# Ai00-X/ai00_server

Hardware: NVIDIA H100
Metric: decode tokens/s RWKV-6-World-7B fp16 batch=16 (higher is better)
Workload: dtype f16

## Files before the change

ai00_server_b200/csrc/wkv.cuh:

```cuda
#pragma once
#include "common.cuh"

namespace b200 {

constexpr int WKV_N = 64;
constexpr float GN_EPS = 64e-5f;

struct WkvParams {
    int version;
    int ld;
    MetaView meta;
    float* state;
    int H;
    const float* r;
    const float* k;
    const float* v;
    const float* g;
    const float* w;
    const float* w_static;
    const float* u;
    const float* lnx_w;
    const float* lnx_b;
    const float* a;
    const float* nu;
    float* v_first;
    int layer0;
    const float* k_k;
    const float* k_a;
    const float* r_k;
    __half* out;
    int kq_tile;
    const __half* wd2t;
    const float* decay_bias;
    const __half* d1;
    int d1_kq;
    int Dd;
    unsigned long long* trace;
};

struct WkvShared {
    float r[WKV_N], k[WKV_N], v[WKV_N], w[WKV_N], b[WKV_N], o[WKV_N];
    float red[4];
};

template <int VER, int KC = 8, bool SPLIT = false>
__device__ __forceinline__ void wkv_slot(const WkvParams& p, const int h, const int t0, const int nt, float (&m)[4][KC],
                                         WkvShared& sm, const float* w_local, const int lt0, const float* pre = nullptr,
                                         const int pre_stride = 0, const float* statics = nullptr) {
    const int tid = (int)threadIdx.x;
    constexpr int LANES = WKV_N / KC;
    const int ig = tid / LANES;
    const int j4 = tid % LANES;
    const int ch = h * WKV_N;
    float u4[KC];
#pragma unroll
    for (int f = 0; f < KC; ++f) u4[f] = 0.f;
    if (VER != 7) {
#pragma unroll
        for (int f = 0; f < KC; ++f) u4[f] = statics ? statics[2 * WKV_N + j4 * KC + f] : p.u[ch + j4 * KC + f];
    }
    for (int tt = 0; tt < nt; ++tt) {
        const int t = t0 + tt;
        const size_t row = (size_t)t * p.ld + ch;
        if (tid < WKV_N) {
            const int c = tid;
            const int pi = (lt0 + tt) * WKV_N + c;
            float r = pre ? pre[pi] : p.r[row + c];
            float k = pre ? pre[pre_stride + pi] : p.k[row + c];
            float v = pre ? pre[2 * pre_stride + pi] : p.v[row + c];
            float w;
            if (VER == 5) w = p.w_static[ch + c];
            else if (w_local) w = w_local[pi];
            else w = pre ? pre[4 * pre_stride + pi] : p.w[row + c];
            if (VER == 7) {
                const float a = pre ? pre[5 * pre_stride + pi] : p.a[row + c];
                float kk = k * p.k_k[ch + c];
                float ss = warp_sum(kk * kk);
                if ((tid & 31) == 0) sm.red[tid >> 5] = ss;
                asm volatile("bar.sync 2, 64;" ::: "memory");
                ss = sm.red[0] + sm.red[1];
                kk = kk / fmaxf(sqrtf(ss), 1e-12f);
                k = k * (1.f + (a - 1.f) * p.k_a[ch + c]);
                if (p.layer0) p.v_first[row + c] = v;
                else v = v + (p.v_first[row + c] - v) * (pre ? pre[6 * pre_stride + pi] : p.nu[row + c]);
                float bonus = warp_sum(r * k * p.r_k[ch + c]);
                if ((tid & 31) == 0) sm.red[2 + (tid >> 5)] = bonus;
                sm.b[c] = kk * a;
                sm.o[c] = -kk;
            }
            sm.r[c] = r; sm.k[c] = k; sm.v[c] = v; sm.w[c] = w;
        }
        __syncthreads();

        float rr[KC], kk_[KC], ww[KC];
#pragma unroll
        for (int f = 0; f < KC; ++f) { rr[f] = sm.r[j4 * KC + f]; kk_[f] = sm.k[j4 * KC + f]; ww[f] = sm.w[j4 * KC + f]; }
        float o[4];
        if (VER != 7) {
#pragma unroll
            for (int e = 0; e < 4; ++e) {
                const float vv = sm.v[ig * 4 + e];
                float* me = m[e];
                float acc = 0.f;
#pragma unroll
                for (int f = 0; f < KC; ++f) {
                    const float kv = kk_[f] * vv;
                    acc += rr[f] * (u4[f] * kv + me[f]);
                    me[f] = kv + ww[f] * me[f];
                }
                o[e] = acc;
            }
        } else {
            float nk[KC], ka[KC];
#pragma unroll
            for (int f = 0; f < KC; ++f) { nk[f] = sm.o[j4 * KC + f]; ka[f] = sm.b[j4 * KC + f]; }
            float sa[4];
#pragma unroll
            for (int e = 0; e < 4; ++e) {
                const float* me = m[e];
                float s_ = 0.f;
#pragma unroll
                for (int f = 0; f < KC; f += 4) s_ += (me[f] * nk[f] + me[f + 1] * nk[f + 1]) + (me[f + 2] * nk[f + 2] + me[f + 3] * nk[f + 3]);
                sa[e] = s_;
            }
#pragma unroll
            for (int off = LANES / 2; off > 0; off >>= 1)
#pragma unroll
                for (int e = 0; e < 4; ++e) sa[e] += __shfl_xor_sync(0xffffffffu, sa[e], off);
#pragma unroll
            for (int e = 0; e < 4; ++e) {
                const float vv = sm.v[ig * 4 + e];
                float* me = m[e];
                float acc = 0.f;
#pragma unroll
                for (int f = 0; f < KC; ++f) {
                    me[f] = me[f] * ww[f] + sa[e] * ka[f] + vv * kk_[f];
                    acc += me[f] * rr[f];
                }
                o[e] = acc;
            }
        }
#pragma unroll
        for (int off = LANES / 2; off > 0; off >>= 1)
#pragma unroll
            for (int e = 0; e < 4; ++e) o[e] += __shfl_xor_sync(0xffffffffu, o[e], off);
        __syncthreads();
        if (j4 == 0) {
#pragma unroll
            for (int e = 0; e < 4; ++e) sm.o[ig * 4 + e] = o[e];
        }
        __syncthreads();

        if (tid < 32) {
            const float x0 = sm.o[tid], x1 = sm.o[tid + 32];
            const float mean = warp_sum(x0 + x1) * (1.f / WKV_N);
            const float d0 = x0 - mean, d1 = x1 - mean;
            const float var = warp_sum(d0 * d0 + d1 * d1) * (1.f / WKV_N);
            const float rstd = 1.0f / sqrtf(var + GN_EPS);
            const float lw0 = statics ? statics[tid] : p.lnx_w[ch + tid], lw1 = statics ? statics[tid + 32] : p.lnx_w[ch + tid + 32];
            const float lb0 = statics ? statics[WKV_N + tid] : p.lnx_b[ch + tid];
            const float lb1 = statics ? statics[WKV_N + tid + 32] : p.lnx_b[ch + tid + 32];
            float y0 = d0 * rstd * lw0 + lb0;
            float y1 = d1 * rstd * lw1 + lb1;
            if (VER == 7) {
                const float bonus = sm.red[2] + sm.red[3];
                y0 += bonus * sm.v[tid];
                y1 += bonus * sm.v[tid + 32];
            }
            const int gi = (lt0 + tt) * WKV_N + tid;
            y0 *= pre ? pre[3 * pre_stride + gi] : p.g[row + tid];
            y1 *= pre ? pre[3 * pre_stride + gi + 32] : p.g[row + tid + 32];
            if (SPLIT) {
                __half h0, l0, h1, l1;
                split_h(y0, h0, l0);
                split_h(y1, h1, l1);
                p.out[a16_index(t, ch + tid, p.kq_tile)] = h0;
                p.out[a16_index(t, ch + tid + 32, p.kq_tile)] = h1;
                p.out[a16_index(t + 16, ch + tid, p.kq_tile)] = l0;
                p.out[a16_index(t + 16, ch + tid + 32, p.kq_tile)] = l1;
            } else {
                p.out[a16_index(t, ch + tid, p.kq_tile)] = f2h_sat(y0);
                p.out[a16_index(t, ch + tid + 32, p.kq_tile)] = f2h_sat(y1);
            }
        }
        __syncthreads();
    }
}

constexpr int WKV_SA_THREADS = 128;
constexpr int WKV_SA_KC = 8;
constexpr int WKV_STAGE_TOK = 4;
constexpr int WKV_STAGE_ARRAYS = 7;

__host__ __device__ inline int wkv_stage_arrays(int ver, bool fold) { return ver == 7 ? 7 : ((ver == 6 && !fold) ? 5 : 4); }

__host__ __device__ inline size_t wkv_smem_bytes(int ver, bool fold, int Dd, int max_tokens, bool split = false) {
    size_t b = 0;
    (void)max_tokens;
    if (fold) b += (size_t)WKV_N * Dd * 2 + (size_t)WKV_STAGE_TOK * WKV_N * 4 + ((((size_t)WKV_STAGE_TOK * Dd * 2 * (split ? 2 : 1)) + 15) & ~(size_t)15) + 2 * WKV_N * 4;
    b += (size_t)wkv_stage_arrays(ver, fold) * WKV_STAGE_TOK * WKV_N * 4 + 3 * WKV_N * 4 + 64;
    return b;
}

template <int VER, bool SPLIT = false>
__global__ void __launch_bounds__(WKV_SA_THREADS, 7) wkv_kernel(const __grid_constant__ WkvParams p, const int max_tokens) {
    constexpr int KC = WKV_SA_KC, LANES = WKV_N / KC, NT = WKV_SA_THREADS;
    __shared__ WkvShared sm;
    extern __shared__ __align__(16) uint8_t wkv_dyn[];
    trace_stamp(p.trace, 0);
    pdl_launch_dependents();
    const int si = blockIdx.y;
    const int h = blockIdx.x;
    const int tid = threadIdx.x;
    const int ig = tid / LANES, j4 = tid % LANES;
    const int ch = h * WKV_N;
    const bool fold = (VER == 6) && p.wd2t != nullptr;
    const int Dd = fold ? p.Dd : 0;
    uint8_t* dyn = wkv_dyn;
    __half* wt = reinterpret_cast<__half*>(dyn);
    float* wl = nullptr;
    __half* ds = nullptr;
    float* part = nullptr;
    if (fold) {
        wl = reinterpret_cast<float*>(dyn + (size_t)WKV_N * Dd * 2);
        ds = reinterpret_cast<__half*>(wl + (size_t)WKV_STAGE_TOK * WKV_N);
        part = reinterpret_cast<float*>(reinterpret_cast<uint8_t*>(ds) + ((((size_t)WKV_STAGE_TOK * Dd * 2 * (SPLIT ? 2 : 1)) + 15) & ~(size_t)15));
        dyn = reinterpret_cast<uint8_t*>(part + 2 * WKV_N);
    }
    const int na = wkv_stage_arrays(VER, fold);
    float* pre_s = reinterpret_cast<float*>(dyn);
    float* statics = pre_s + na * WKV_STAGE_TOK * WKV_N;
    if (fold) {
        const uint4* src = reinterpret_cast<const uint4*>(p.wd2t + (size_t)h * WKV_N * Dd);
        uint4* dst = reinterpret_cast<uint4*>(wt);
        for (int i = tid; i < WKV_N * Dd / 8; i += NT) dst[i] = src[i];
    }
    for (int i = tid; i < 3 * WKV_N; i += NT) {
        const int a = i >> 6, c = i & (WKV_N - 1);
        float v = 0.f;
        if (a == 0) v = p.lnx_w[ch + c];
        else if (a == 1) v = p.lnx_b[ch + c];
        else if (VER != 7) v = p.u[ch + c];
        statics[i] = v;
    }
    const float bias = fold ? p.decay_bias[ch + (tid & (WKV_N - 1))] : 0.f;
    const int nslots = p.meta.nslots();
    const bool live = si < nslots;
    const int slot = live ? p.meta.slot_id()[si] : 0;
    const int t0 = live ? p.meta.slot_start()[si] : 0;
    const int nt = live ? p.meta.slot_count()[si] : 0;
    float* M = p.state + ((size_t)slot * p.H + h) * (WKV_N * WKV_N);
    float m[4][KC];
    if (live) {
#pragma unroll
        for (int e = 0; e < 4; ++e)
#pragma unroll
            for (int q = 0; q < KC / 4; ++q) {
                const float4 v4 = __ldcs(reinterpret_cast<const float4*>(M + (ig * 4 + e) * WKV_N + j4 * KC + q * 4));
                m[e][q * 4] = v4.x; m[e][q * 4 + 1] = v4.y; m[e][q * 4 + 2] = v4.z; m[e][q * 4 + 3] = v4.w;
            }
    }
    pdl_wait();
    trace_stamp(p.trace, 1);
    if (!live) return;

    const bool staged = nt <= WKV_STAGE_TOK;
    if (staged) {
        constexpr int UMAX = WKV_STAGE_ARRAYS * WKV_STAGE_TOK * WKV_N / NT;
        const int per = nt * WKV_N, total = na * per;
        const int ndd = fold ? nt * Dd : 0;
#pragma unroll
        for (int half = 0; half < 2; ++half) {
            float val[UMAX / 2];
#pragma unroll
            for (int u = 0; u < UMAX / 2; ++u) {
                const int i = tid + (half * (UMAX / 2) + u) * NT;
                val[u] = 0.f;
                if (i < total) {
                    const int a = i / per, rem = i - a * per;
                    const size_t at = (size_t)(t0 + (rem >> 6)) * p.ld + ch + (rem & (WKV_N - 1));
                    const float* src = a == 0 ? p.r : a == 1 ? p.k : a == 2 ? p.v : a == 3 ? p.g : a == 4 ? p.w : a == 5 ? p.a : p.nu;
                    if (src) val[u] = src[at];
                }
            }
#pragma unroll
            for (int u = 0; u < UMAX / 2; ++u) {
                const int i = tid + (half * (UMAX / 2) + u) * NT;
                if (i < total) {
                    const int a = i / per, rem = i - a * per;
                    pre_s[a * (WKV_STAGE_TOK * WKV_N) + rem] = val[u];
                }
            }
        }
        for (int i = tid; i < ndd; i += NT) {
            const int tt = i / Dd;
            ds[i] = p.d1[a16_index(t0 + tt, i - tt * Dd, p.d1_kq)];
        }
        if (SPLIT)
            for (int i = tid; i < ndd; i += NT) {
                const int tt = i / Dd;
                ds[WKV_STAGE_TOK * Dd + i] = p.d1[a16_index(t0 + tt + 16, i - tt * Dd, p.d1_kq)];
            }
    }

    auto fold_token = [&](const __half* dt, const int slot_tok) {
        const int c = tid & (WKV_N - 1), qk = tid >> 6;
        const int kq0 = qk * (Dd >> 1), kq1 = kq0 + (Dd >> 1);
        float acc0 = 0.f, acc1 = 0.f;
        if (SPLIT) {
            const __half* dl = dt + WKV_STAGE_TOK * Dd;
            for (int k = kq0; k < kq1; k += 2) {
                acc0 = fmaf(__half2float(wt[k * WKV_N + c]), __half2float(dt[k]) + __half2float(dl[k]), acc0);
                acc1 = fmaf(__half2float(wt[(k + 1) * WKV_N + c]), __half2float(dt[k + 1]) + __half2float(dl[k + 1]), acc1);
            }
        } else {
            for (int k = kq0; k < kq1; k += 2) {
                acc0 = fmaf(__half2float(wt[k * WKV_N + c]), __half2float(dt[k]), acc0);
                acc1 = fmaf(__half2float(wt[(k + 1) * WKV_N + c]), __half2float(dt[k + 1]), acc1);
            }
        }
        part[qk * WKV_N + c] = acc0 + acc1;
        __syncthreads();
        if (tid < WKV_N) wl[slot_tok * WKV_N + c] = expf(-expf(bias + (part[c] + part[WKV_N + c])));
    };
    if (staged || !fold) {
        if (fold)
            for (int tt = 0; tt < nt; ++tt) {
                __syncthreads();
                fold_token(ds + tt * Dd, tt);
            }
        __syncthreads();
        wkv_slot<VER, KC, SPLIT>(p, h, t0, nt, m, sm, fold ? wl : nullptr, 0, staged ? pre_s : nullptr, WKV_STAGE_TOK * WKV_N, statics);
    } else {
        for (int tt = 0; tt < nt; ++tt) {
            __syncthreads();
            for (int k = tid; k < Dd; k += NT) ds[k] = p.d1[a16_index(t0 + tt, k, p.d1_kq)];
            if (SPLIT)
                for (int k = tid; k < Dd; k += NT) ds[WKV_STAGE_TOK * Dd + k] = p.d1[a16_index(t0 + tt + 16, k, p.d1_kq)];
            __syncthreads();
            fold_token(ds, 0);
            __syncthreads();
            wkv_slot<VER, KC, SPLIT>(p, h, t0 + tt, 1, m, sm, wl, 0, nullptr, WKV_STAGE_TOK * WKV_N, statics);
        }
    }
#pragma unroll
    for (int e = 0; e < 4; ++e)
#pragma unroll
        for (int q = 0; q < KC / 4; ++q)
            __stcs(reinterpret_cast<float4*>(M + (ig * 4 + e) * WKV_N + j4 * KC + q * 4),
                   make_float4(m[e][q * 4], m[e][q * 4 + 1], m[e][q * 4 + 2], m[e][q * 4 + 3]));
    trace_stamp(p.trace, 7);
}

}
```

Baseline: 2192.

## Interleave WKV shared-memory columns and stream per-column operands to cut registers

Stores r/k/w/b and the bonus u in shared memory with a permuted column index, so each lane reads stride-LANES columns without bank conflicts. The state update now loops over columns and reads those operands from shared memory one at a time instead of holding whole per-lane arrays in registers. The staging loader becomes a rolled loop with a small buffer, and launch bounds go from 7 to 8 blocks per SM to raise occupancy. This trades more shared-memory loads inside the inner loop for lower register pressure.

```diff
diff --git a/ai00_server_b200/csrc/wkv.cuh b/ai00_server_b200/csrc/wkv.cuh
--- a/ai00_server_b200/csrc/wkv.cuh
+++ b/ai00_server_b200/csrc/wkv.cuh
@@ -5,6 +5,7 @@
 
 constexpr int WKV_N = 64;
 constexpr float GN_EPS = 64e-5f;
+constexpr int WKV_STAGE_TOK = 4;
 
 struct WkvParams {
     int version;
@@ -38,6 +39,8 @@
     unsigned long long* trace;
 };
 
+__device__ __forceinline__ int wkv_kcol(const int c) { return (c & 7) * 8 + (c >> 3); }
+
 struct WkvShared {
     float r[WKV_N], k[WKV_N], v[WKV_N], w[WKV_N], b[WKV_N], o[WKV_N];
     float red[4];
@@ -45,35 +48,30 @@
 
 template <int VER, int KC = 8, bool SPLIT = false>
 __device__ __forceinline__ void wkv_slot(const WkvParams& p, const int h, const int t0, const int nt, float (&m)[4][KC],
-                                         WkvShared& sm, const float* w_local, const int lt0, const float* pre = nullptr,
-                                         const int pre_stride = 0, const float* statics = nullptr) {
+                                         WkvShared& sm, const float* w_local, const float* pre, const bool staged,
+                                         const float* statics) {
     const int tid = (int)threadIdx.x;
     constexpr int LANES = WKV_N / KC;
     const int ig = tid / LANES;
     const int j4 = tid % LANES;
     const int ch = h * WKV_N;
-    float u4[KC];
-#pragma unroll
-    for (int f = 0; f < KC; ++f) u4[f] = 0.f;
-    if (VER != 7) {
-#pragma unroll
-        for (int f = 0; f < KC; ++f) u4[f] = statics ? statics[2 * WKV_N + j4 * KC + f] : p.u[ch + j4 * KC + f];
-    }
+    const bool fold = VER == 6 && p.wd2t != nullptr;
+    constexpr int PS = WKV_STAGE_TOK * WKV_N;
     for (int tt = 0; tt < nt; ++tt) {
         const int t = t0 + tt;
         const size_t row = (size_t)t * p.ld + ch;
         if (tid < WKV_N) {
-            const int c = tid;
-            const int pi = (lt0 + tt) * WKV_N + c;
-            float r = pre ? pre[pi] : p.r[row + c];
-            float k = pre ? pre[pre_stride + pi] : p.k[row + c];
-            float v = pre ? pre[2 * pre_stride + pi] : p.v[row + c];
+            const int c = tid, kc = wkv_kcol(c);
+            const int pi = tt * WKV_N + c;
+            float r = staged ? pre[pi] : p.r[row + c];
+            float k = staged ? pre[PS + pi] : p.k[row + c];
+            float v = staged ? pre[2 * PS + pi] : p.v[row + c];
             float w;
             if (VER == 5) w = p.w_static[ch + c];
-            else if (w_local) w = w_local[pi];
-            else w = pre ? pre[4 * pre_stride + pi] : p.w[row + c];
+            else if (fold) w = w_local[pi];
+            else w = staged ? pre[4 * PS + pi] : p.w[row + c];
             if (VER == 7) {
-                const float a = pre ? pre[5 * pre_stride + pi] : p.a[row + c];
+                const float a = staged ? pre[5 * PS + pi] : p.a[row + c];
                 float kk = k * p.k_k[ch + c];
                 float ss = warp_sum(kk * kk);
                 if ((tid & 31) == 0) sm.red[tid >> 5] = ss;
@@ -82,62 +80,55 @@
                 kk = kk / fmaxf(sqrtf(ss), 1e-12f);
                 k = k * (1.f + (a - 1.f) * p.k_a[ch + c]);
                 if (p.layer0) p.v_first[row + c] = v;
-                else v = v + (p.v_first[row + c] - v) * (pre ? pre[6 * pre_stride + pi] : p.nu[row + c]);
+                else v = v + (p.v_first[row + c] - v) * (staged ? pre[6 * PS + pi] : p.nu[row + c]);
                 float bonus = warp_sum(r * k * p.r_k[ch + c]);
                 if ((tid & 31) == 0) sm.red[2 + (tid >> 5)] = bonus;
-                sm.b[c] = kk * a;
-                sm.o[c] = -kk;
-            }
-            sm.r[c] = r; sm.k[c] = k; sm.v[c] = v; sm.w[c] = w;
-        }
-        __syncthreads();
-
-        float rr[KC], kk_[KC], ww[KC];
-#pragma unroll
-        for (int f = 0; f < KC; ++f) { rr[f] = sm.r[j4 * KC + f]; kk_[f] = sm.k[j4 * KC + f]; ww[f] = sm.w[j4 * KC + f]; }
-        float o[4];
+                sm.b[kc] = kk * a;
+                sm.o[kc] = -kk;
+            }
+            sm.r[kc] = r; sm.k[kc] = k; sm.v[c] = v; sm.w[kc] = w;
+        }
+        __syncthreads();
+
+        float o[4], vv[4];
+#pragma unroll
+        for (int e = 0; e < 4; ++e) { o[e] = 0.f; vv[e] = sm.v[ig * 4 + e]; }
         if (VER != 7) {
 #pragma unroll
-            for (int e = 0; e < 4; ++e) {
-                const float vv = sm.v[ig * 4 + e];
-                float* me = m[e];
-                float acc = 0.f;
-#pragma unroll
-                for (int f = 0; f < KC; ++f) {
-                    const float kv = kk_[f] * vv;
-                    acc += rr[f] * (u4[f] * kv + me[f]);
-                    me[f] = kv + ww[f] * me[f];
+            for (int f = 0; f < KC; ++f) {
+                const int c = f * LANES + j4;
+                const float rf = sm.r[c], kf = sm.k[c], wf = sm.w[c], uf = statics[2 * WKV_N + c];
+#pragma unroll
+                for (int e = 0; e < 4; ++e) {
+                    const float kv = kf * vv[e];
+                    o[e] += rf * (uf * kv + m[e][f]);
+                    m[e][f] = kv + wf * m[e][f];
                 }
-                o[e] = acc;
             }
         } else {
-            float nk[KC], ka[KC];
-#pragma unroll
-            for (int f = 0; f < KC; ++f) { nk[f] = sm.o[j4 * KC + f]; ka[f] = sm.b[j4 * KC + f]; }
             float sa[4];
 #pragma unroll
-            for (int e = 0; e < 4; ++e) {
-                const float* me = m[e];
-                float s_ = 0.f;
-#pragma unroll
-                for (int f = 0; f < KC; f += 4) s_ += (me[f] * nk[f] + me[f + 1] * nk[f + 1]) + (me[f + 2] * nk[f + 2] + me[f + 3] * nk[f + 3]);
-                sa[e] = s_;
+            for (int e = 0; e < 4; ++e) sa[e] = 0.f;
+#pragma unroll
+            for (int f = 0; f < KC; f += 4) {
+                const int c = f * LANES + j4;
+                const float n0 = sm.o[c], n1 = sm.o[c + LANES], n2 = sm.o[c + 2 * LANES], n3 = sm.o[c + 3 * LANES];
+#pragma unroll
+                for (int e = 0; e < 4; ++e) sa[e] += (m[e][f] * n0 + m[e][f + 1] * n1) + (m[e][f + 2] * n2 + m[e][f + 3] * n3);
             }
 #pragma unroll
             for (int off = LANES / 2; off > 0; off >>= 1)
 #pragma unroll
                 for (int e = 0; e < 4; ++e) sa[e] += __shfl_xor_sync(0xffffffffu, sa[e], off);
 #pragma unroll
-            for (int e = 0; e < 4; ++e) {
-                const float vv = sm.v[ig * 4 + e];
-                float* me = m[e];
-                float acc = 0.f;
-#pragma unroll
-                for (int f = 0; f < KC; ++f) {
-                    me[f] = me[f] * ww[f] + sa[e] * ka[f] + vv * kk_[f];
-                    acc += me[f] * rr[f];
+            for (int f = 0; f < KC; ++f) {
+                const int c = f * LANES + j4;
+                const float rf = sm.r[c], kf = sm.k[c], wf = sm.w[c], kaf = sm.b[c];
+#pragma unroll
+                for (int e = 0; e < 4; ++e) {
+                    m[e][f] = m[e][f] * wf + sa[e] * kaf + vv[e] * kf;
+                    o[e] += m[e][f] * rf;
                 }
-                o[e] = acc;
             }
         }
 #pragma unroll
@@ -157,9 +148,8 @@
             const float d0 = x0 - mean, d1 = x1 - mean;
             const float var = warp_sum(d0 * d0 + d1 * d1) * (1.f / WKV_N);
             const float rstd = 1.0f / sqrtf(var + GN_EPS);
-            const float lw0 = statics ? statics[tid] : p.lnx_w[ch + tid], lw1 = statics ? statics[tid + 32] : p.lnx_w[ch + tid + 32];
-            const float lb0 = statics ? statics[WKV_N + tid] : p.lnx_b[ch + tid];
-            const float lb1 = statics ? statics[WKV_N + tid + 32] : p.lnx_b[ch + tid + 32];
+            const float lw0 = statics[tid], lw1 = statics[tid + 32];
+            const float lb0 = statics[WKV_N + tid], lb1 = statics[WKV_N + tid + 32];
             float y0 = d0 * rstd * lw0 + lb0;
             float y1 = d1 * rstd * lw1 + lb1;
             if (VER == 7) {
@@ -167,9 +157,9 @@
                 y0 += bonus * sm.v[tid];
                 y1 += bonus * sm.v[tid + 32];
             }
-            const int gi = (lt0 + tt) * WKV_N + tid;
-            y0 *= pre ? pre[3 * pre_stride + gi] : p.g[row + tid];
-            y1 *= pre ? pre[3 * pre_stride + gi + 32] : p.g[row + tid + 32];
+            const int gi = tt * WKV_N + tid;
+            y0 *= staged ? pre[3 * PS + gi] : p.g[row + tid];
+            y1 *= staged ? pre[3 * PS + gi + 32] : p.g[row + tid + 32];
             if (SPLIT) {
                 __half h0, l0, h1, l1;
                 split_h(y0, h0, l0);
@@ -189,8 +179,6 @@
 
 constexpr int WKV_SA_THREADS = 128;
 constexpr int WKV_SA_KC = 8;
-constexpr int WKV_STAGE_TOK = 4;
-constexpr int WKV_STAGE_ARRAYS = 7;
 
 __host__ __device__ inline int wkv_stage_arrays(int ver, bool fold) { return ver == 7 ? 7 : ((ver == 6 && !fold) ? 5 : 4); }
 
@@ -203,7 +191,7 @@
 }
 
 template <int VER, bool SPLIT = false>
-__global__ void __launch_bounds__(WKV_SA_THREADS, 7) wkv_kernel(const __grid_constant__ WkvParams p, const int max_tokens) {
+__global__ void __launch_bounds__(WKV_SA_THREADS, 8) wkv_kernel(const __grid_constant__ WkvParams p, const int max_tokens) {
     constexpr int KC = WKV_SA_KC, LANES = WKV_N / KC, NT = WKV_SA_THREADS;
     __shared__ WkvShared sm;
     extern __shared__ __align__(16) uint8_t wkv_dyn[];
@@ -216,19 +204,12 @@
     const int ch = h * WKV_N;
     const bool fold = (VER == 6) && p.wd2t != nullptr;
     const int Dd = fold ? p.Dd : 0;
-    uint8_t* dyn = wkv_dyn;
-    __half* wt = reinterpret_cast<__half*>(dyn);
-    float* wl = nullptr;
-    __half* ds = nullptr;
-    float* part = nullptr;
-    if (fold) {
-        wl = reinterpret_cast<float*>(dyn + (size_t)WKV_N * Dd * 2);
-        ds = reinterpret_cast<__half*>(wl + (size_t)WKV_STAGE_TOK * WKV_N);
-        part = reinterpret_cast<float*>(reinterpret_cast<uint8_t*>(ds) + ((((size_t)WKV_STAGE_TOK * Dd * 2 * (SPLIT ? 2 : 1)) + 15) & ~(size_t)15));
-        dyn = reinterpret_cast<uint8_t*>(part + 2 * WKV_N);
-    }
+    __half* wt = reinterpret_cast<__half*>(wkv_dyn);
+    float* wl = reinterpret_cast<float*>(wkv_dyn + (size_t)WKV_N * Dd * 2);
+    __half* ds = reinterpret_cast<__half*>(wl + (size_t)WKV_STAGE_TOK * WKV_N);
+    float* part = reinterpret_cast<float*>(reinterpret_cast<uint8_t*>(ds) + ((((size_t)WKV_STAGE_TOK * Dd * 2 * (SPLIT ? 2 : 1)) + 15) & ~(size_t)15));
     const int na = wkv_stage_arrays(VER, fold);
-    float* pre_s = reinterpret_cast<float*>(dyn);
+    float* pre_s = fold ? part + 2 * WKV_N : reinterpret_cast<float*>(wkv_dyn);
     float* statics = pre_s + na * WKV_STAGE_TOK * WKV_N;
     if (fold) {
         const uint4* src = reinterpret_cast<const uint4*>(p.wd2t + (size_t)h * WKV_N * Dd);
@@ -241,7 +222,7 @@
         if (a == 0) v = p.lnx_w[ch + c];
         else if (a == 1) v = p.lnx_b[ch + c];
         else if (VER != 7) v = p.u[ch + c];
-        statics[i] = v;
+        statics[a == 2 ? 2 * WKV_N + wkv_kcol(c) : i] = v;
     }
     const float bias = fold ? p.decay_bias[ch + (tid & (WKV_N - 1))] : 0.f;
     const int nslots = p.meta.nslots();
@@ -266,15 +247,15 @@
 
     const bool staged = nt <= WKV_STAGE_TOK;
     if (staged) {
-        constexpr int UMAX = WKV_STAGE_ARRAYS * WKV_STAGE_TOK * WKV_N / NT;
         const int per = nt * WKV_N, total = na * per;
         const int ndd = fold ? nt * Dd : 0;
-#pragma unroll
-        for (int half = 0; half < 2; ++half) {
-            float val[UMAX / 2];
-#pragma unroll
-            for (int u = 0; u < UMAX / 2; ++u) {
-                const int i = tid + (half * (UMAX / 2) + u) * NT;
+        constexpr int UB = 4;
+#pragma unroll 1
+        for (int i0 = 0; i0 < total; i0 += UB * NT) {
+            float val[UB];
+#pragma unroll
+            for (int u = 0; u < UB; ++u) {
+                const int i = i0 + tid + u * NT;
                 val[u] = 0.f;
                 if (i < total) {
                     const int a = i / per, rem = i - a * per;
@@ -284,8 +265,8 @@
                 }
             }
 #pragma unroll
-            for (int u = 0; u < UMAX / 2; ++u) {
-                const int i = tid + (half * (UMAX / 2) + u) * NT;
+            for (int u = 0; u < UB; ++u) {
+                const int i = i0 + tid + u * NT;
                 if (i < total) {
                     const int a = i / per, rem = i - a * per;
                     pre_s[a * (WKV_STAGE_TOK * WKV_N) + rem] = val[u];
@@ -330,7 +311,7 @@
                 fold_token(ds + tt * Dd, tt);
             }
         __syncthreads();
-        wkv_slot<VER, KC, SPLIT>(p, h, t0, nt, m, sm, fold ? wl : nullptr, 0, staged ? pre_s : nullptr, WKV_STAGE_TOK * WKV_N, statics);
+        wkv_slot<VER, KC, SPLIT>(p, h, t0, nt, m, sm, wl, pre_s, staged, statics);
     } else {
         for (int tt = 0; tt < nt; ++tt) {
             __syncthreads();
@@ -340,7 +321,7 @@
             __syncthreads();
             fold_token(ds, 0);
             __syncthreads();
-            wkv_slot<VER, KC, SPLIT>(p, h, t0 + tt, 1, m, sm, wl, 0, nullptr, WKV_STAGE_TOK * WKV_N, statics);
+            wkv_slot<VER, KC, SPLIT>(p, h, t0 + tt, 1, m, sm, wl, pre_s, false, statics);
         }
     }
 #pragma unroll
```

Measured after the change: 2199 (median of 6 runs). No clear change (+0.3%).
